# springmeyer/cov-tiles

Hardware: AMD Instinct MI355X
Metric: GB/s raw COVT bytes decoded + Mvertices/s, z2–z14 tile batch, 1/2/4/8 GPU (higher is better)
Workload: dtype int32

## Files before the change

cov-tiles_amd/__init__.py:

```python
from __future__ import annotations

import ctypes as C
import os
import subprocess
from dataclasses import dataclass
from typing import List, Optional

import numpy as np

_HERE = os.path.dirname(os.path.abspath(__file__))
_LIB = os.path.join(_HERE, os.environ.get("COVT_LIB_VARIANT", "libcovt.so"))

OK = 0
ERR_UNSUPPORTED_ENCODING = -1
ERR_TRUNCATED = -2
ERR_COUNT_MISMATCH = -3
ERR_BAD_HEADER = -4
ERR_DEVICE = -5
ERR_INVALID_ARG = -6
INPUT_PADDING = 4096
FORMAT_GENC, FORMAT_GEND = 0, 1
FAMILY_RLE, FAMILY_VARINT, FAMILY_FASTPFOR, FAMILY_LANE, FAMILY_SPLIT, FAMILY_SPLIT_FPF, FAMILY_SPLIT_RLE = range(7)
NUM_FAMILIES = 7
DESC_LANE, DESC_SPLIT, DESC_SPLIT_PAD, DESC_SPLIT_FPF = 0x1, 0x2, 0x4, 0x8
DESC_SPLIT_RLE = 0x10
SPLIT_SLOTS = 8
ID_FORMAT, ID_JAVA = 0, 1
LAUNCH_AUTO, LAUNCH_FUSED, LAUNCH_FORKED = 0, 1, 2
LAUNCH_FPF_STREAM, LAUNCH_FPF_CLASSIC = 0x4, 0x8

(OP_NONE, OP_BYTE_RLE_U8, OP_RLE_U64, OP_RLE_I32, OP_RLE_S64, OP_VARINT_I32, OP_VARINT_ZZ_I32,
 OP_VARINT_ZZ_DELTA_I32, OP_VARINT_ZZ_DELTA_XY, OP_VARINT_DELTA_MORTON, OP_FPF_ZZ_DELTA_I32, OP_FPF_ZZ_DELTA_XY,
 OP_FPF_DELTA_MORTON, OP_VARINT_U64, OP_VARINT_I32_AS_I64, OP_VARINT_ZZ_DELTA_I64, OP_BYTE_RLE_RAW,
 OP_VARINT_ZZ_I32_AS_I64, OP_VARINT_ZZ_S64, OP_VARINT_ZZ_DELTA_S64) = range(20)

PLAN_PROPERTIES = 0x1
RELEASE_PINNED = 0x2
PROP_BOOLEAN, PROP_INT64, PROP_FLOAT, PROP_STRING = 0, 1, 2, 3
PROP_DICT_OWNER, PROP_DENSE_BOOL, PROP_UNSUPPORTED, PROP_DATA_SHORT, PROP_UNSUPPORTED_LATE = 0x1, 0x2, 0x4, 0x8, 0x10

GEOMETRY_TYPES, GEOMETRY_OFFSETS, PART_OFFSETS, RING_OFFSETS, VERTEX_OFFSETS, VERTEX_BUFFER = range(4, 10)


class CovtError(Exception):
    status = 0


class IllegalArgumentException(CovtError, ValueError):
    pass


class ArrayIndexOutOfBoundsException(CovtError, IndexError):
# ... 1007 lines not shown
```

cov-tiles_amd/csrc/covt_decode.hip:

```cpp
#include <hip/hip_runtime.h>
#include <stdint.h>

#include "covt.h"
#include "covt_internal.h"
#include "covt_wave.h"
#include "covt_walk.h"

namespace covt {

constexpr int kWin = 1024;
constexpr int kFpfBlock = 256;
constexpr int kFpfPage = 65536;
constexpr int kFpfBcCap = 3 * kFpfPage / kFpfBlock + kFpfPage;

#ifndef COVT_LONG_STREAM
#define COVT_LONG_STREAM 16384
#endif
#ifndef COVT_LONG_PRIO
#define COVT_LONG_PRIO 2
#endif
#ifndef COVT_RLE_SHORT_SPAN
#define COVT_RLE_SHORT_SPAN 448
#endif
#ifndef COVT_CHUNK_PRIO
// ... 2039 lines not shown
    if ((cx | cy) == 0u) return;
    __builtin_amdgcn_s_waitcnt(0x0f70);
    int32_t* o = (int32_t*)out;
    typedef __attribute__((address_space(1))) i32x4 g_i4;
    const int32_t nq = (v1 - v0) >> 2;
    const int32_t last = v0 + 4 * (nq > 0 ? nq - 1 : 0);
    constexpr int kDeep = 8;
    for (int32_t q0 = 0; q0 < nq; q0 += 64 * kDeep) {
        i32x4 v[kDeep];
#pragma unroll
        for (int k = 0; k < kDeep; ++k) v[k] = *(const g_i4*)(o + min(v0 + 4 * (q0 + 64 * k + lane_id()), last));
#pragma unroll
        for (int k = 0; k < kDeep; ++k) {
            const int32_t q = q0 + 64 * k + lane_id();
            if (q < nq)
                st_out16(o + v0 + 4 * q, make_int4((int32_t)((uint32_t)v[k].x + cx), (int32_t)((uint32_t)v[k].y + cy),
                                                   (int32_t)((uint32_t)v[k].z + cx), (int32_t)((uint32_t)v[k].w + cy)));
        }
    }
    const int32_t i = v0 + 4 * nq + lane_id();
    if (i < v1) o[i] = (int32_t)((uint32_t)o[i] + (((i - v0) & 1) ? cy : cx));
}

constexpr int kSplitSlots = COVT_SPLIT_SLOTS;
struct Agg {
    int32_t cnt;
    uint32_t sx, sy;
};
__device__ __forceinline__ Agg agg_cat(const Agg& a, const Agg& b, bool xy) {
    if (a.cnt < 0) return a;
    if (b.cnt < 0) return Agg{b.cnt, b.sx, (uint32_t)a.cnt + b.sy};
    const bool sw = xy && (a.cnt & 1);
    return Agg{a.cnt + b.cnt, a.sx + (sw ? b.sy : b.sx), a.sy + (sw ? b.sx : b.sy)};
}
typedef __attribute__((address_space(1))) uint64_t g_u64;
__device__ __forceinline__ void rec_publish(covt_stream_result* rec, const Agg& a, uint32_t tag) {
    if (lane_id() == 0) {
        g_u64* g = (g_u64*)rec;
        const uint64_t t = (uint64_t)tag << 32;
        __hip_atomic_store(g, t | (uint32_t)a.cnt, __ATOMIC_RELAXED, __HIP_MEMORY_SCOPE_AGENT);
        __hip_atomic_store(g + 1, t | a.sx, __ATOMIC_RELAXED, __HIP_MEMORY_SCOPE_AGENT);
        __hip_atomic_store(g + 2, t | a.sy, __ATOMIC_RELAXED, __HIP_MEMORY_SCOPE_AGENT);
    }
}
__device__ __forceinline__ bool rec_try(covt_stream_result* rec, uint32_t tag, Agg& a) {
    g_u64* g = (g_u64*)rec;
// ... 298 lines not shown
                                                                           covt_stream_result* __restrict__ res) {
    constexpr int kStride = K == kSplitFpf ? kFamSmemFpf : K == kSplitRle ? kFamSmemRle : kFamSmemVarint;
    __shared__ __attribute__((aligned(16))) uint8_t smem[kWavesPerBlock * kStride];
    const int wv = uni((int)(threadIdx.x >> 6));
#ifdef COVT_TIMING
    const uint64_t t_start = __builtin_amdgcn_s_memrealtime();
#endif
    const int64_t t = decode_split_chunk<K>((WaveSmem*)(smem + wv * kStride), in, descs, n_chunks, out, res);
#ifdef COVT_TIMING
    if (t >= 0 && covt_phase_buf && lane_id() == 0) {
        const uint64_t t_end = __builtin_amdgcn_s_memrealtime();
        uint32_t* row = covt_phase_buf + (descs + kSplitSlots * t - covt_phase_desc0) * kPhases;
        row[0] = (uint32_t)(t_end - t_start);
        row[1] = (uint32_t)t_start;
    }
#else
    (void)t;
#endif
}

template <int FAM, bool FS = false>
__device__ __forceinline__ void decode_family_wave(uint8_t* smem, const uint8_t* __restrict__ in,
                                                   const covt_stream_desc* __restrict__ descs, int64_t sid,
                                                   uint8_t* __restrict__ out, covt_stream_result* __restrict__ res) {
    const covt_stream_desc d = descs[sid];
    if ((d.flags & (COVT_DESC_LANE | COVT_DESC_SPLIT | COVT_DESC_SPLIT_PAD)) || op_family(d.op) != FAM) return;
    if (d.byte_length > kLongStream || d.num_values > kLongStream) __builtin_amdgcn_s_setprio(COVT_LONG_PRIO);
#ifdef COVT_TIMING
    const uint64_t t_start = __builtin_amdgcn_s_memrealtime();
#endif
    Ctx c;
    c.sm = (WaveSmem*)smem;
    c.sb = in + d.in_off;
    c.out = out + d.out_off;
    c.avail = d.avail;
    c.n = d.num_values;
    c.nb = d.num_bits;
    c.op = d.op;
    c.byte_length = d.byte_length;
    c.err = 0;
    c.consumed = 0;
#ifdef COVT_TIMING
    c.ph_last = __builtin_amdgcn_s_memtime();
    for (int k = 0; k < kPhases; ++k) c.ph[k] = 0;
#endif
    if (c.n < 0 || c.avail < 0 || c.byte_length < 0) {
        c.err = COVT_ERR_INVALID_ARG;
    } else if (FAM == COVT_FAMILY_RLE) {
        if (c.op == COVT_OP_BYTE_RLE_U8 || c.op == COVT_OP_BYTE_RLE_RAW) { if (c.n > 0) run_rle_byte(c); }
// ... 40 lines not shown
        r.status = c.err;
        r.consumed = c.consumed;
#ifdef COVT_TIMING
        const uint64_t t_end = __builtin_amdgcn_s_memrealtime();
        r.status = c.err ? -1 : (int32_t)(t_end - t_start);
        r.consumed = (int32_t)(uint32_t)t_start;
        if (covt_phase_buf)
            for (int k = 0; k < kPhases; ++k) covt_phase_buf[(descs + sid - covt_phase_desc0) * kPhases + k] = c.ph[k];
#endif
        res[sid] = r;
    }
}

#ifndef COVT_FPF_WAVES
#define COVT_FPF_WAVES 7
#endif
#ifndef COVT_FPF_STREAM_WAVES
#define COVT_FPF_STREAM_WAVES 8
#endif
template <int FAM, bool FS = false>
__global__ __launch_bounds__(64 * kWavesPerBlock) __attribute__((amdgpu_waves_per_eu(FAM == COVT_FAMILY_FASTPFOR ? (FS ? COVT_FPF_STREAM_WAVES : COVT_FPF_WAVES) : 7))) void decode_family_kernel(const uint8_t* __restrict__ in,
                                                            const covt_stream_desc* __restrict__ descs,
                                                            int64_t n_streams, uint8_t* __restrict__ out,
                                                            covt_stream_result* __restrict__ res) {
    constexpr int kStride = FAM == COVT_FAMILY_RLE ? kFamSmemRle
                            : FAM == COVT_FAMILY_VARINT ? kFamSmemVarint : kFamSmemFpf;
    __shared__ __attribute__((aligned(16))) uint8_t smem[kWavesPerBlock * kStride];
    const int wv = uni((int)(threadIdx.x >> 6));
    const int64_t sid = (int64_t)blockIdx.x * kWavesPerBlock + wv;
    if (sid >= n_streams) return;
    decode_family_wave<FAM, FS>(smem + wv * kStride, in, descs, sid, out, res);
}

#ifndef COVT_LANE_SLOT
#define COVT_LANE_SLOT 17
#endif
constexpr int kLaneSlot = COVT_LANE_SLOT;
static_assert(kLaneSlot % 4 == 1, "16-byte granules plus one dword");
struct LaneBytes {
    const uint8_t* sb;
    uint32_t* slot;
    int32_t avail;
    int32_t w0;
    int32_t cq;
    uint32_t cw;
    __device__ __forceinline__ void load(int32_t p) {
        const uintptr_t a = (uintptr_t)(sb + p), a4 = a & ~(uintptr_t)3;
        w0 = p - (int32_t)(a & 3u);
        const int32_t need = avail - w0;
        uint32_t st[kLaneSlot];
#pragma unroll
        for (int k = 0; k < kLaneSlot / 4; ++k) {
            u32x4 v = {0u, 0u, 0u, 0u};
            if (16 * k < need) v = *(const __attribute__((address_space(1))) u32x4*)(a4 + 16 * k);
// ... 335 lines not shown
        sg.n[f] = counts[f];
        off += counts[f];
    }
    uint64_t wg = 0;
    for (int k = 0; k < COVT_NUM_FAMILIES; ++k) {
        const int f = covt::kFusedOrder[k];
        const int64_t n = f == COVT_FAMILY_SPLIT || f == COVT_FAMILY_SPLIT_FPF || f == COVT_FAMILY_SPLIT_RLE
                              ? counts[f] / covt::kSplitSlots : counts[f];
        const int64_t per = f == COVT_FAMILY_LANE ? 64 * kWavesPerBlock : kWavesPerBlock;
        wg += (uint64_t)((n + per - 1) / per);
        if (wg > 0x7fffffffull) return COVT_ERR_INVALID_ARG;
        sg.wg_end[k] = (uint32_t)wg;
    }
    if (wg == 0) return COVT_OK;
    hipLaunchKernelGGL(covt::decode_fused_kernel, dim3((unsigned)wg), dim3(64 * kWavesPerBlock), 0, stream,
                       d_in, d_out, sg);
    return hipGetLastError() == hipSuccess ? COVT_OK : COVT_ERR_DEVICE;
}

extern "C" int covt_launch_family_split_mode(int fam, const uint8_t* d_in, const covt_stream_desc* d_desc,
                                             int64_t n_streams, uint8_t* d_out, covt_stream_result* d_res,
                                             const covt_stream_desc* d_split, int64_t n_split,
                                             covt_stream_result* d_split_res, hipStream_t stream, int fpf_mode) {
    if (fpf_mode != 0 && fpf_mode != COVT_LAUNCH_FPF_STREAM && fpf_mode != COVT_LAUNCH_FPF_CLASSIC)
        return COVT_ERR_INVALID_ARG;
    if (n_split < 0 || n_split % covt::kSplitSlots) return COVT_ERR_INVALID_ARG;
    if (n_split && fam != COVT_FAMILY_VARINT && fam != COVT_FAMILY_FASTPFOR && fam != COVT_FAMILY_RLE)
        return COVT_ERR_INVALID_ARG;
    if (n_streams <= 0 && n_split == 0) return COVT_OK;
    if (n_streams < 0) n_streams = 0;
    if (fam == COVT_FAMILY_LANE) {
        const int64_t lblocks = (n_streams + 255) / 256;
        if (lblocks > 0x7fffffff) return COVT_ERR_INVALID_ARG;
        hipLaunchKernelGGL(covt::decode_lane_kernel, dim3((unsigned)lblocks), dim3(256), 0, stream, d_in, d_desc,
                           n_streams, d_out, d_res);
        return hipGetLastError() == hipSuccess ? COVT_OK : COVT_ERR_DEVICE;
    }
    const int64_t n_chunks = n_split / covt::kSplitSlots;
    const dim3 block(64 * kWavesPerBlock);
    if (n_chunks > 0) {
        const int64_t sblocks = (n_chunks + kWavesPerBlock - 1) / kWavesPerBlock;
        if (sblocks > 0x7fffffff) return COVT_ERR_INVALID_ARG;
        if (fam == COVT_FAMILY_FASTPFOR)
            hipLaunchKernelGGL(covt::decode_split_kernel<covt::kSplitFpf>, dim3((unsigned)sblocks), block, 0, stream,
                               d_in, d_split, n_chunks, d_out, d_split_res);
        else if (fam == COVT_FAMILY_RLE)
            hipLaunchKernelGGL(covt::decode_split_kernel<covt::kSplitRle>, dim3((unsigned)sblocks), block, 0, stream,
                               d_in, d_split, n_chunks, d_out, d_split_res);
        else
            hipLaunchKernelGGL(covt::decode_split_kernel<covt::kSplitVarint>, dim3((unsigned)sblocks), block, 0,
                               stream, d_in, d_split, n_chunks, d_out, d_split_res);
        if (hipGetLastError() != hipSuccess) return COVT_ERR_DEVICE;
    }
    if (n_streams <= 0) return COVT_OK;
    const int64_t blocks = (n_streams + kWavesPerBlock - 1) / kWavesPerBlock;
    if (blocks > 0x7fffffff) return COVT_ERR_INVALID_ARG;
    const dim3 grid((unsigned)blocks);
    switch (fam) {
    case COVT_FAMILY_RLE:
        hipLaunchKernelGGL(covt::decode_family_kernel<COVT_FAMILY_RLE>, grid, block, 0, stream, d_in, d_desc,
                           n_streams, d_out, d_res);
        break;
    case COVT_FAMILY_VARINT:
        hipLaunchKernelGGL(covt::decode_family_kernel<COVT_FAMILY_VARINT>, grid, block, 0, stream, d_in, d_desc,
                           n_streams, d_out, d_res);
        break;
    case COVT_FAMILY_FASTPFOR:
        if (fpf_mode == COVT_LAUNCH_FPF_STREAM || (fpf_mode == 0 && n_streams >= kFpfStreamMinStreams))
            hipLaunchKernelGGL((covt::decode_family_kernel<COVT_FAMILY_FASTPFOR, true>), grid, block, 0, stream, d_in,
                               d_desc, n_streams, d_out, d_res);
        else
            hipLaunchKernelGGL((covt::decode_family_kernel<COVT_FAMILY_FASTPFOR, false>), grid, block, 0, stream, d_in,
                               d_desc, n_streams, d_out, d_res);
        break;
    default: return COVT_ERR_INVALID_ARG;
    }
    return hipGetLastError() == hipSuccess ? COVT_OK : COVT_ERR_DEVICE;
}

extern "C" int covt_launch_family_split(int fam, const uint8_t* d_in, const covt_stream_desc* d_desc,
                                        int64_t n_streams, uint8_t* d_out, covt_stream_result* d_res,
                                        const covt_stream_desc* d_split, int64_t n_split, covt_stream_result* d_split_res,
                                        hipStream_t stream) {
    return covt_launch_family_split_mode(fam, d_in, d_desc, n_streams, d_out, d_res, d_split, n_split, d_split_res,
                                         stream, 0);
}

extern "C" int covt_launch_family(int fam, const uint8_t* d_in, const covt_stream_desc* d_desc, int64_t n_streams,
                                  uint8_t* d_out, covt_stream_result* d_res, hipStream_t stream) {
    return covt_launch_family_split(fam, d_in, d_desc, n_streams, d_out, d_res, nullptr, 0, nullptr, stream);
}

extern "C" int covt_op_family_of(int op) { return covt::op_family(op); }

#ifdef COVT_TIMING
extern "C" int covt_debug_set_phase_buffer(void* d_buf, const void* d_desc0) {
    if (hipMemcpyToSymbol(HIP_SYMBOL(covt::covt_phase_desc0), &d_desc0, sizeof(d_desc0)) != hipSuccess) return -5;
    return hipMemcpyToSymbol(HIP_SYMBOL(covt::covt_phase_buf), &d_buf, sizeof(d_buf)) == hipSuccess ? 0 : -5;
}
#endif
```

cov-tiles_amd/csrc/covt_host.cpp:

```cpp
#include <hip/hip_runtime.h>

#include <algorithm>
#include <atomic>
#include <cstdlib>
#include <cstring>
#include <sys/mman.h>
#include <memory>
#include <mutex>
#include <numeric>
#include <thread>
#include <unordered_map>
#include <vector>

#include "covt.h"
#include "covt_internal.h"
#include "covt_walk.h"
#include "covt_props_plan.h"

namespace {

bool name_is(const uint8_t* t, int64_t off, int64_t len, const char* s) {
    return (size_t)len == std::strlen(s) && std::memcmp(t + off, s, (size_t)len) == 0;
}

// ... 469 lines not shown
                return f;
            }
    }
    auto* f = new ForkCtx();
    f->device = dev;
    bool ok = true;
    for (int i = 0; i < kForkAux && ok; ++i)
        ok = hipStreamCreateWithFlags(&f->aux[i], hipStreamNonBlocking) == hipSuccess &&
             hipEventCreateWithFlags(&f->join[i], hipEventDisableTiming) == hipSuccess;
    if (ok) ok = hipEventCreateWithFlags(&f->fork, hipEventDisableTiming) == hipSuccess;
    if (!ok) {
        fork_destroy(f);
        return nullptr;
    }
    return f;
}
void fork_release(ForkCtx* f) {
    std::lock_guard<std::mutex> g(g_fork_mu);
    g_fork_free.push_back(f);
}

int launch_grouped(const uint8_t* d_in, const covt_stream_desc* d_desc, const int64_t counts[COVT_NUM_FAMILIES],
                   uint8_t* d_out, covt_stream_result* d_res, hipStream_t s, int mode = COVT_LAUNCH_AUTO) {
    const int fpf_mode = mode & (COVT_LAUNCH_FPF_STREAM | COVT_LAUNCH_FPF_CLASSIC);
    mode &= ~(COVT_LAUNCH_FPF_STREAM | COVT_LAUNCH_FPF_CLASSIC);
    if (fpf_mode == (COVT_LAUNCH_FPF_STREAM | COVT_LAUNCH_FPF_CLASSIC)) return COVT_ERR_INVALID_ARG;
    if (mode != COVT_LAUNCH_AUTO && mode != COVT_LAUNCH_FUSED && mode != COVT_LAUNCH_FORKED) return COVT_ERR_INVALID_ARG;
    int dev = 0;
    if (hipGetDevice(&dev) != hipSuccess) return COVT_ERR_DEVICE;
    if (s) {
        int sdev = -1;
        if (hipStreamGetDevice(s, &sdev) != hipSuccess || sdev != dev) return COVT_ERR_DEVICE;
    }
    ForkCtx* fp = fork_acquire(dev);
    if (!fp) return COVT_ERR_DEVICE;
    struct Back { ForkCtx* f; ~Back() { fork_release(f); } } back{fp};
    ForkCtx& f = *fp;
    int64_t off[COVT_NUM_FAMILIES];
    off[0] = 0;
    for (int k = 1; k < COVT_NUM_FAMILIES; ++k) off[k] = off[k - 1] + counts[k - 1];
    constexpr int kSplitV = COVT_FAMILY_SPLIT, kSplitF = COVT_FAMILY_SPLIT_FPF, kSplitR = COVT_FAMILY_SPLIT_RLE;
    const int64_t n_split = counts[kSplitV] + counts[kSplitF] + counts[kSplitR];
    const bool splits = n_split > 0;
    auto n_of = [&](int fam) { return fam < 0 ? 0 : counts[fam]; };
    struct Q {
        int fam[3];
    };
    Q qs[4];
    int nq = 0;
    auto add = [&](int a, int b2, int c3) {
        Q q{{-1, -1, -1}};
        int k = 0;
        for (int f : {a, b2, c3})
            if (n_of(f) > 0) q.fam[k++] = f;
        if (k) qs[nq++] = q;
    };
    if (splits && hipMemsetAsync(d_res + off[kSplitV], 0, (size_t)n_split * sizeof(covt_stream_result), s) != hipSuccess)
        return COVT_ERR_DEVICE;
    {
        const int64_t waves = n_split / COVT_SPLIT_SLOTS + counts[COVT_FAMILY_FASTPFOR] + counts[COVT_FAMILY_RLE] +
                              counts[COVT_FAMILY_VARINT] +
                              (counts[COVT_FAMILY_LANE] + kFusedLaneStreams - 1) / kFusedLaneStreams;
        if (mode == COVT_LAUNCH_FUSED || (mode == COVT_LAUNCH_AUTO && waves <= kFusedMaxWaves))
            return covt_launch_fused(d_in, d_desc, counts, d_out, d_res, s);
    }
    if (splits) {
        add(kSplitV, COVT_FAMILY_VARINT, kSplitR);
        add(COVT_FAMILY_FASTPFOR, -1, -1);
        add(COVT_FAMILY_RLE, COVT_FAMILY_LANE, -1);
        add(kSplitF, -1, -1);
    } else {
        for (int f : {COVT_FAMILY_FASTPFOR, COVT_FAMILY_VARINT, COVT_FAMILY_RLE, COVT_FAMILY_LANE}) add(f, -1, -1);
    }
    if (nq > 1 && hipEventRecord(f.fork, s) != hipSuccess) return COVT_ERR_DEVICE;
    int st = COVT_OK;
    int nforked = 0;
    for (int i = 0; i < nq && !st; ++i) {
        hipStream_t q = s;
        if (i > 0) {
            q = f.aux[i - 1];
            if (hipStreamWaitEvent(q, f.fork, 0) != hipSuccess) return COVT_ERR_DEVICE;
            nforked = i;
        }
        for (int k = 0; k < 3 && !st; ++k) {
            const int fam = qs[i].fam[k];
            if (fam < 0) continue;
            if (fam != kSplitV && fam != kSplitF && fam != kSplitR) {
                st = covt_launch_family_split_mode(fam, d_in, d_desc + off[fam], counts[fam], d_out, d_res + off[fam],
                                                   nullptr, 0, nullptr, q, fpf_mode);
                continue;
            }
            const int kind = fam == kSplitV ? COVT_FAMILY_VARINT : fam == kSplitR ? COVT_FAMILY_RLE : COVT_FAMILY_FASTPFOR;
            st = covt_launch_family_split(kind, d_in, nullptr, 0, d_out, nullptr, d_desc + off[fam], counts[fam],
                                          d_res + off[fam], q);
        }
    }
    for (int i = 0; i < nforked; ++i) {
        if (hipEventRecord(f.join[i], f.aux[i]) != hipSuccess) return COVT_ERR_DEVICE;
        if (hipStreamWaitEvent(s, f.join[i], 0) != hipSuccess) return COVT_ERR_DEVICE;
    }
    return st;
}

}

namespace {

struct Prefault {
    std::vector<std::thread> th;
// ... 1254 lines not shown
```

cov-tiles_amd/csrc/covt_internal.h:

```cpp
#ifndef COVT_INTERNAL_H
#define COVT_INTERNAL_H

#include <hip/hip_runtime.h>
#include <stdint.h>

#include "covt.h"

extern "C" {
int covt_launch_family(int fam, const uint8_t* d_in, const covt_stream_desc* d_desc, int64_t n_streams,
                       uint8_t* d_out, covt_stream_result* d_res, hipStream_t stream);
int covt_launch_family_split(int fam, const uint8_t* d_in, const covt_stream_desc* d_desc, int64_t n_streams,
                             uint8_t* d_out, covt_stream_result* d_res, const covt_stream_desc* d_split,
                             int64_t n_split, covt_stream_result* d_split_res, hipStream_t stream);
int covt_launch_family_split_mode(int fam, const uint8_t* d_in, const covt_stream_desc* d_desc, int64_t n_streams,
                                  uint8_t* d_out, covt_stream_result* d_res, const covt_stream_desc* d_split,
                                  int64_t n_split, covt_stream_result* d_split_res, hipStream_t stream, int fpf_mode);
int covt_op_family_of(int op);
int covt_launch_fused(const uint8_t* d_in, const covt_stream_desc* d_desc, const int64_t counts[COVT_NUM_FAMILIES],
                      uint8_t* d_out, covt_stream_result* d_res, hipStream_t stream);
}
constexpr int64_t kFpfStreamMinStreams = 65536;
constexpr int64_t kFusedMaxWaves = 4096;
#ifndef COVT_WAVES_PER_BLOCK
#define COVT_WAVES_PER_BLOCK 2
#endif
constexpr int kWavesPerBlock = COVT_WAVES_PER_BLOCK;
constexpr int64_t kFusedLaneStreams = 64 * kWavesPerBlock;

constexpr int64_t kOutAlign = 128;
__host__ __device__ inline int64_t align_out(int64_t x) { return (x + kOutAlign - 1) & ~(kOutAlign - 1); }

constexpr int kLaunchFamShift = 13;
__host__ __device__ inline uint32_t lane_op_index(int32_t op) {
    return op == COVT_OP_BYTE_RLE_U8 ? 0u : op == COVT_OP_RLE_U64 ? 1u : op == COVT_OP_RLE_I32 ? 2u
         : op == COVT_OP_RLE_S64 ? 3u : 4u;
}
__host__ __device__ inline uint32_t launch_key(uint32_t fam, bool lane, int32_t op, int64_t cost) {
    const uint64_t c = cost > 0 ? (uint64_t)cost : 0;
    uint32_t sub;
    if (lane) {
        sub = (lane_op_index(op) << 10) | (1023u - (uint32_t)(c < 1023 ? c : 1023));
    } else {
        uint32_t h = 0;
        if (c) {
// ... 57 lines not shown
```

include/covt.h:

```cpp
#ifndef COVT_H
#define COVT_H

#include <stddef.h>
#include <stdint.h>

#ifdef __cplusplus
extern "C" {
#endif

#define COVT_OK 0
#define COVT_ERR_UNSUPPORTED_ENCODING (-1)
#define COVT_ERR_TRUNCATED (-2)
#define COVT_ERR_COUNT_MISMATCH (-3)
#define COVT_ERR_BAD_HEADER (-4)
#define COVT_ERR_DEVICE (-5)
#define COVT_ERR_INVALID_ARG (-6)

#define COVT_INPUT_PADDING 4096

#define COVT_FORMAT_GENC 0
#define COVT_FORMAT_GEND 1

#define COVT_ID_FORMAT 0
#define COVT_ID_JAVA 1
// ... 121 lines not shown
                     int32_t n_tiles, int32_t format, int32_t id_mode, covt_plan** out);
void covt_plan_destroy(covt_plan* plan);
int64_t covt_plan_num_streams(const covt_plan* plan);
int64_t covt_plan_output_bytes(const covt_plan* plan);
int covt_plan_totals(const covt_plan* plan, int64_t* in_bytes, int64_t* out_bytes, int64_t* vertices);
int covt_plan_streams(const covt_plan* plan, covt_stream_info* out);
int64_t covt_plan_num_descs(const covt_plan* plan);
int covt_plan_descs(const covt_plan* plan, covt_stream_desc* out);
int covt_plan_desc_streams(const covt_plan* plan, int64_t* out);
int covt_plan_family_counts(const covt_plan* plan, int64_t counts[COVT_NUM_FAMILIES]);
int covt_plan_tile_status(const covt_plan* plan, int32_t* out);

int covt_decode_streams_device(const uint8_t* d_in, const covt_stream_desc* d_desc, int64_t n_streams,
                               uint8_t* d_out, covt_stream_result* d_res, void* hip_stream);

int covt_decode_streams_device_grouped(const uint8_t* d_in, const covt_stream_desc* d_desc,
                                       const int64_t family_counts[COVT_NUM_FAMILIES], uint8_t* d_out,
                                       covt_stream_result* d_res, void* hip_stream);
#define COVT_LAUNCH_AUTO 0
#define COVT_LAUNCH_FUSED 1
#define COVT_LAUNCH_FORKED 2
#define COVT_LAUNCH_FPF_STREAM 0x4
#define COVT_LAUNCH_FPF_CLASSIC 0x8
int covt_decode_streams_device_grouped_mode(const uint8_t* d_in, const covt_stream_desc* d_desc,
                                            const int64_t family_counts[COVT_NUM_FAMILIES], uint8_t* d_out,
                                            covt_stream_result* d_res, void* hip_stream, int32_t launch_mode);

int covt_plan_decode_host(const covt_plan* plan, const uint8_t* bytes, uint64_t n_bytes, uint8_t* host_out,
                          covt_stream_result* host_res);

int covt_plan_decode_host_multi(const covt_plan* plan, const uint8_t* bytes, uint64_t n_bytes, int32_t n_gpus,
                                uint8_t* host_out, covt_stream_result* host_res);

int covt_plan_decode_host_shards(const covt_plan* plan, const uint8_t* bytes, uint64_t n_bytes, int32_t n_shards,
                                 const int32_t* shard_devices, uint8_t* host_out, covt_stream_result* host_res);

int covt_plan_release_device(const covt_plan* plan);

#define COVT_GEOM_CLOSED_IN_STREAM 0x1u
#define COVT_GEOM_TOO_LARGE 0x80000000u

typedef struct covt_geom_desc {
    int64_t in_off[6];
    int32_t in_len[6];
    int32_t in_res[6];
    int64_t out_off[6];
// ... 136 lines not shown
```

Before: 610.6.

## Add cooperative multi-wave FastPFOR decode for large streams with auto launch selection

Adds a FastPFOR kernel where a whole workgroup of several waves decodes one large stream. Wave 0 parses page and block headers into shared LDS batches, and all waves then unpack 256-value blocks and apply exceptions in parallel. The host launcher picks this path automatically when the FastPFOR family is small and there are no split FPF streams, and schedules it first on the forked queues. The aim is to cut the tail latency of single large FastPFOR streams decoded by one wave. The cost is workgroup barriers, serialized header parsing on one wave, and higher LDS use per workgroup.

```diff
diff --git a/cov-tiles_amd/__init__.py b/cov-tiles_amd/__init__.py
--- a/cov-tiles_amd/__init__.py
+++ b/cov-tiles_amd/__init__.py
@@ -28,6 +28,7 @@
 ID_FORMAT, ID_JAVA = 0, 1
 LAUNCH_AUTO, LAUNCH_FUSED, LAUNCH_FORKED = 0, 1, 2
 LAUNCH_FPF_STREAM, LAUNCH_FPF_CLASSIC = 0x4, 0x8
+LAUNCH_FPF_COOP, LAUNCH_FPF_NOCOOP = 0x10, 0x20
 
 (OP_NONE, OP_BYTE_RLE_U8, OP_RLE_U64, OP_RLE_I32, OP_RLE_S64, OP_VARINT_I32, OP_VARINT_ZZ_I32,
  OP_VARINT_ZZ_DELTA_I32, OP_VARINT_ZZ_DELTA_XY, OP_VARINT_DELTA_MORTON, OP_FPF_ZZ_DELTA_I32, OP_FPF_ZZ_DELTA_XY,
diff --git a/cov-tiles_amd/csrc/covt_decode.hip b/cov-tiles_amd/csrc/covt_decode.hip
--- a/cov-tiles_amd/csrc/covt_decode.hip
+++ b/cov-tiles_amd/csrc/covt_decode.hip
@@ -2085,6 +2085,409 @@
     if (i < v1) o[i] = (int32_t)((uint32_t)o[i] + (((i - v0) & 1) ? cy : cx));
 }
 
+#ifndef COVT_FPF_COOP_WAVES
+#define COVT_FPF_COOP_WAVES 8
+#endif
+constexpr int kCoopWaves = COVT_FPF_COOP_WAVES;
+static_assert(kCoopWaves >= 2 && kCoopWaves <= 16, "cooperative FastPFOR workgroup: 2..16 waves");
+struct __attribute__((aligned(16))) CoopSmem {
+    WaveSmem w0;
+    uint32_t stage[kCoopWaves][328];
+    uint32_t patch[kCoopWaves][256];
+    int32_t rb[64], rce[64], ridx[64], rpk[64], rbcoff[64];
+    uint32_t rxcur[64];
+    int32_t xs[64];
+    uint32_t tot[2][kCoopWaves][2];
+    int32_t page[4];
+    int32_t bat[4];
+};
+static_assert(2 * sizeof(CoopSmem) <= 160 * 1024 && sizeof(CoopSmem) <= 64 * 1024,
+              "two cooperative FastPFOR workgroups per CU (160 KiB of LDS)");
+
+template <int OP>
+__device__ __forceinline__ void run_fastpfor_coop(Ctx& c, CoopSmem& cs, const int w) {
+    WaveSmem& sm = cs.w0;
+    const int l = lane_id();
+    const Words W{c.sb, c.byte_length / 4};
+    const int32_t nw32 = W.nw;
+    const uint32_t sbmis = (uint32_t)((uintptr_t)c.sb & 15);
+    const uint32_t bsel = be_sel(sbmis & 3u);
+    const g_u8* sb4 = (const g_u8*)(((uintptr_t)c.sb) & ~(uintptr_t)3);
+    Carry cr{0u, 0u};
+    uint32_t sc = 0;
+    int32_t L = 0, p = 1, done = 0, mw0 = 0;
+    int xs_v = 0, xz_v = -1, xc_v = 0;
+    uint32_t head1 = 0;
+    if (w == 0) {
+        if (c.byte_length > c.avail) c.err = COVT_ERR_TRUNCATED;
+        if (!c.err && nw32 > 0) {
+            const uint32_t head0 = W.uniform(0);
+            head1 = W.uniform(1);
+            L = (int32_t)head0;
+            if (L < 0) c.err = COVT_ERR_BAD_HEADER;
+            L -= L % kFpfBlock;
+            if (!c.err && L > c.n) c.err = COVT_ERR_COUNT_MISMATCH;
+        }
+    }
+    const uintptr_t s_end = (uintptr_t)c.sb + 4u * (uint32_t)nw32;
+    struct WordsRaw {
+        uint4 r;
+        int32_t base;
+        uint32_t sh;
+    };
+    auto words_issue = [&](int32_t wd) -> WordsRaw {
+        const uintptr_t addr = (uintptr_t)c.sb + 4u * (uint32_t)wd;
+        const uintptr_t a16 = addr & ~(uintptr_t)15;
+        const uint32_t o = (uint32_t)(addr & 15u);
+        const uint32_t lmax = s_end > a16 ? (uint32_t)((s_end - 1 - a16) >> 4) : 0u;
+        WordsRaw q;
+        q.r = ld128_off((const g_u8*)a16, 16u * min((uint32_t)l, lmax));
+        q.base = uni(wd - (int32_t)(o >> 2));
+        q.sh = o & 3u;
+        return q;
+    };
+    auto words_store = [&](uint32_t* dst, const WordsRaw& q) -> int32_t {
+        const uint32_t nx = lane_next(q.r.x);
+        const uint32_t sel = be_sel(q.sh);
+        const int32_t wl = q.base + 4 * l;
+        uint4 wv;
+        wv.x = wl < nw32 ? be_word(q.r.y, q.r.x, sel) : 0u;
+        wv.y = wl + 1 < nw32 ? be_word(q.r.z, q.r.y, sel) : 0u;
+        wv.z = wl + 2 < nw32 ? be_word(q.r.w, q.r.z, sel) : 0u;
+        wv.w = wl + 3 < nw32 ? be_word(nx, q.r.w, sel) : 0u;
+        wave_sync();
+        ((uint4*)dst)[l] = wv;
+        wave_sync();
+        return q.base;
+    };
+    auto load_words = [&](uint32_t* dst, int32_t wd) -> int32_t { return words_store(dst, words_issue(wd)); };
+    int32_t ie = 0, nblocks = 0, bclen = 0, bc = 0, cbase = 0, cur = 0, pk = 0;
+    bool xin = false;
+    auto chunk_load = [&](int32_t at) { cbase = (int32_t)(4 * (load_words(sm.u.f.cbuf, bc + (at >> 2)) - bc)); };
+    for (;;) {
+        if (w == 0) {
+            int32_t go = 0;
+            do {
+                if (c.err || nw32 <= 0 || done >= L) break;
+                done = uni(done);
+                const int32_t thissize = uni((L - done) < kFpfPage ? (L - done) : kFpfPage);
+                const int32_t p0 = uni(p);
+                if (p0 >= nw32) { c.err = COVT_ERR_TRUNCATED; break; }
+                const int64_t ie0 = (int64_t)p0 + (int32_t)(p0 == 1 ? head1 : W.uniform(p0));
+                if (ie0 < 0 || ie0 >= nw32) { c.err = COVT_ERR_TRUNCATED; break; }
+                ie = (int32_t)ie0;
+                mw0 = load_words(sm.u.f.cbuf, ie);
+                auto mword = [&](int32_t wd) -> uint32_t { return uniu(sm.u.f.cbuf[wd - mw0]); };
+                const int32_t bytesize = (int32_t)mword(ie++);
+                if (bytesize < 0 || bytesize > kFpfBcCap) { c.err = COVT_ERR_BAD_HEADER; break; }
+                xc_v = 0;
+                const int32_t bcw = (bytesize + 3) / 4;
+                bc = ie;
+                if (bc + bcw >= nw32) { c.err = COVT_ERR_TRUNCATED; break; }
+                ie += bcw;
+                int64_t ie64 = ie;
+                {
+                    int32_t dbase = INT32_MIN / 2;
+                    auto dword = [&](int32_t wd) -> uint32_t {
+                        if (wd >= mw0 && wd < mw0 + 255) return mword(wd);
+                        if (wd < dbase || wd >= dbase + 255) dbase = load_words(sm.u.f.ring, wd);
+                        return uniu(sm.u.f.ring[wd - dbase]);
+                    };
+                    uint32_t bm = dword((int32_t)ie64++) & ~1u;
+                    xs_v = 0;
+                    xz_v = -1;
+                    while (bm) {
+                        const int32_t k = __builtin_ctz(bm) + 1;
+                        bm &= bm - 1;
+                        if (ie64 >= nw32) { c.err = COVT_ERR_TRUNCATED; break; }
+                        const int32_t size = (int32_t)dword((int32_t)ie64++);
+                        if (size < 0) { c.err = COVT_ERR_BAD_HEADER; break; }
+                        const int64_t groups = ((int64_t)size + 31) / 32;
+                        xs_v = l == k ? (int)(uint32_t)ie64 : xs_v;
+                        xz_v = l == k ? size : xz_v;
+                        ie64 += groups * k;
+                        ie64 -= ((groups * 32 - size) * k) / 32;
+                    }
+                    if (c.err) break;
+                }
+                xin = ie64 - mw0 <= 255;
+                ie = (int32_t)(ie64 < nw32 ? ie64 : (int64_t)nw32);
+                nblocks = uni(thissize / kFpfBlock);
+                bclen = uni(bcw * 4);
+                cbase = (int32_t)(4 * (mw0 - bc));
+                cur = 0;
+                pk = p0 + 1;
+                cs.xs[l] = xs_v;
+                go = 1;
+            } while (false);
+            if (l == 0) {
+                cs.page[0] = go;
+                cs.page[1] = done;
+                cs.page[2] = bc;
+            }
+        }
+        __syncthreads();
+        if (uni(cs.page[0]) == 0) break;
+        const int32_t pdone = uni(cs.page[1]);
+        const g_u8* cbyte = (const g_u8*)(c.sb + 4u * (uint32_t)uni(cs.page[2]));
+        int32_t jbat = 0;
+        for (;;) {
+            if (w == 0) {
+                jbat = uni(jbat);
+                int32_t nbat = uni(min(64, nblocks - jbat));
+                uint32_t hw_v = 0u;
+                int32_t cur_v = bclen + 1;
+                cur = uni(cur);
+                cbase = uni(cbase);
+                if (!xin && cur <= bclen && (uint32_t)(cur - cbase) > (uint32_t)(1020 - 258)) chunk_load(cur);
+                for (int32_t g = 0; g < nbat; ++g) {
+                    cur = uni(cur);
+                    cbase = uni(cbase);
+                    if (cur > bclen) break;
+                    if (!xin && cur - cbase > 1020 - 8) {
+                        nbat = g;
+                        break;
+                    }
+                    const int32_t q = cur - cbase;
+                    const uint32_t hw =
+                        uniu(__builtin_amdgcn_alignbyte(sm.u.f.cbuf[(q >> 2) + 1], sm.u.f.cbuf[q >> 2], (uint32_t)q & 3u));
+                    const int32_t ce = (int32_t)((hw >> 8) & 0xffu);
+                    const int32_t nx = cur + (ce > 0 ? 3 + ce : 2);
+                    if (!xin && g > 0 && nx - cbase > 1020) {
+                        nbat = g;
+                        break;
+                    }
+                    hw_v = l == g ? hw : hw_v;
+                    cur_v = l == g ? cur : cur_v;
+                    cur = nx;
+                }
+                nbat = uni(nbat);
+                const bool in = l < nbat;
+                const int32_t b_v = (int32_t)(int8_t)(hw_v & 0xffu);
+                const int32_t ce_v = (int32_t)((hw_v >> 8) & 0xffu);
+                const bool hasx = ce_v > 0;
+                const int32_t idx_v = hasx ? (int32_t)(int8_t)((hw_v >> 16) & 0xffu) - b_v : 1;
+                const bool arr_k = hasx && idx_v >= 2 && idx_v <= 32;
+                const bool arr = in && arr_k;
+                int32_t xcur_v = 0;
+                for (uint64_t todo = __ballot(arr); todo;) {
+                    const int32_t kk = __builtin_amdgcn_readlane(idx_v, (int32_t)__builtin_ctzll(todo));
+                    const bool mine = arr && idx_v == kk;
+                    const uint32_t v = mine ? (uint32_t)ce_v : 0u;
+                    const uint32_t s = incl_scan(v);
+                    const int32_t base = __builtin_amdgcn_readlane(xc_v, kk);
+                    xcur_v = mine ? base + (int32_t)(s - v) : xcur_v;
+                    xc_v += l == kk ? (int32_t)lane_bcast(s, 63) : 0;
+                    todo &= ~__ballot(mine);
+                }
+                const uint32_t w8 = in ? 8u * (uint32_t)(b_v & 63) : 0u;
+                const uint32_t pinc = incl_scan(w8);
+                const int32_t pk_v = pk + (int32_t)(pinc - w8);
+                pk += (int32_t)lane_bcast(pinc, 63);
+                int32_t nok = nbat;
+                int32_t ferr = nbat == 0 ? COVT_ERR_BAD_HEADER : 0;
+                {
+                    const int32_t xsz = lane_get(xz_v, arr_k ? idx_v : 0);
+                    bool bad = (uint32_t)b_v > 32u || cur_v + 2 > bclen;
+                    bad |= hasx && (cur_v + 3 + ce_v > bclen || (idx_v != 1 && !arr_k));
+                    bad |= arr_k && (xsz < 0 || xcur_v + ce_v > xsz);
+                    const bool trunc = pk_v + 8 * b_v > nw32;
+                    const uint64_t fail = __ballot(in && (bad || trunc));
+                    if (fail) {
+                        nok = (int32_t)__builtin_ctzll(fail);
+                        ferr = __builtin_amdgcn_readlane(bad ? COVT_ERR_BAD_HEADER : COVT_ERR_TRUNCATED, nok);
+                    }
+                }
+                cs.rb[l] = b_v;
+                cs.rce[l] = ce_v;
+                cs.ridx[l] = idx_v;
+                cs.rpk[l] = pk_v;
+                cs.rbcoff[l] = cur_v + (hasx ? 3 : 2);
+                cs.rxcur[l] = (uint32_t)xcur_v;
+                if (ferr) c.err = ferr;
+                if (l == 0) {
+                    cs.bat[0] = jbat;
+                    cs.bat[1] = nok;
+                    cs.bat[2] = ferr;
+                    cs.bat[3] = (ferr != 0 || jbat + nbat >= nblocks) ? 1 : 0;
+                }
+                jbat += nbat;
+            }
+            __syncthreads();
+            const int32_t j0 = uni(cs.bat[0]), nok = uni(cs.bat[1]);
+            const bool last = uni(cs.bat[3]) != 0;
+            struct Pre {
+                uint4 raw;
+                uint32_t pos, x0, x1, x2;
+            };
+            auto issue = [&](int32_t g, Pre& pr) {
+                const int32_t b = uni(cs.rb[g]), ce = uni(cs.rce[g]), k = uni(cs.ridx[g]);
+                const int32_t pkc = uni(cs.rpk[g]), bcoff = uni(cs.rbcoff[g]);
+                const uint32_t xcur = uniu(cs.rxcur[g]);
+                const uintptr_t a16 = ((uintptr_t)c.sb + 4u * (uint32_t)pkc) & ~(uintptr_t)15;
+                pr.raw = ld128_off((const g_u8*)a16, 16u * min((uint32_t)l, 2u * (uint32_t)b + 1u));
+                pr.pos = pr.x0 = pr.x1 = pr.x2 = 0u;
+                if (ce > 0) {
+                    pr.pos = cbyte[(uint32_t)(bcoff + min(l, ce - 1)) ^ 3u];
+                    if (k != 1) {
+                        const uint32_t xs = (uint32_t)uni(cs.xs[k]);
+                        const int32_t wx = (int32_t)(xs + (__umul24(xcur + (uint32_t)l, (uint32_t)k) >> 5));
+                        const uint32_t wi = l < ce && wx < nw32 ? (uint32_t)wx : 0u;
+                        const u32x3 xv = *(const g_v3*)(sb4 + 4u * wi);
+                        pr.x0 = xv.x;
+                        pr.x1 = xv.y;
+                        pr.x2 = xv.z;
+                    }
+                }
+            };
+            Pre pr;
+            pr.raw = make_uint4(0, 0, 0, 0);
+            pr.pos = pr.x0 = pr.x1 = pr.x2 = 0u;
+            if (w < nok) issue(w, pr);
+            for (int32_t g0 = 0; g0 < nok; g0 += kCoopWaves, ++sc) {
+                const int32_t g = g0 + w;
+                const bool act = g < nok;
+                const int64_t vbase = (int64_t)pdone + (int64_t)(j0 + g) * kFpfBlock;
+                uint32_t v[4] = {0u, 0u, 0u, 0u};
+                uint32_t tx = 0u, ty = 0u;
+                if (act) {
+                    const int32_t b = uni(cs.rb[g]), ce = uni(cs.rce[g]), k = uni(cs.ridx[g]);
+                    const int32_t pkc = uni(cs.rpk[g]), bcoff = uni(cs.rbcoff[g]);
+                    const uint32_t xcur = uniu(cs.rxcur[g]);
+                    uint32_t* stage = cs.stage[w];
+                    uint32_t* patch = cs.patch[w];
+                    const uintptr_t a16 = ((uintptr_t)c.sb + 4u * (uint32_t)pkc) & ~(uintptr_t)15;
+                    const uint4 raw = pr.raw;
+                    const bool el = l < ce;
+                    const uint32_t pos = pr.pos, x0 = pr.x0, x1 = pr.x1, x2 = pr.x2;
+                    uint32_t xbit = 0u;
+                    int32_t wx = 0;
+                    if (ce > 0 && k != 1) {
+                        const uint32_t bb = __umul24(xcur + (uint32_t)l, (uint32_t)k);
+                        xbit = bb & 31u;
+                        wx = (int32_t)((uint32_t)uni(cs.xs[k]) + (bb >> 5));
+                    }
+                    const int32_t qoff = (int32_t)(((sbmis + 4u * (uint32_t)pkc) & 15u) >> 2);
+                    {
+                        uint4 raw2 = make_uint4(0, 0, 0, 0);
+                        if (b == 32) raw2 = sld128(a16 + 1024);
+                        const uint32_t nxt = lane_next(raw.x, raw2.x);
+                        uint4 wv;
+                        wv.x = be_word(raw.y, raw.x, bsel);
+                        wv.y = be_word(raw.z, raw.y, bsel);
+                        wv.z = be_word(raw.w, raw.z, bsel);
+                        wv.w = be_word(nxt, raw.w, bsel);
+                        ((uint4*)stage)[l] = wv;
+                        if (b == 32 && l == 0) {
+                            uint4 w2;
+                            w2.x = be_word(raw2.y, raw2.x, bsel);
+                            w2.y = be_word(raw2.z, raw2.y, bsel);
+                            w2.z = be_word(raw2.w, raw2.z, bsel);
+                            w2.w = be_word(0u, raw2.w, bsel);
+                            ((uint4*)stage)[64] = w2;
+                        }
+                    }
+                    if (ce > 0) ((uint4*)patch)[l] = make_uint4(0, 0, 0, 0);
+                    wave_sync();
+                    {
+                        const uint32_t mask = b == 32 ? 0xffffffffu : ((1u << b) - 1u);
+                        uint32_t bit = __umul24((uint32_t)(l & 7) * 4u, (uint32_t)b);
+                        const int32_t wb = (int32_t)__umul24((uint32_t)(l >> 3), (uint32_t)b) + qoff;
+#pragma unroll
+                        for (int q = 0; q < 4; ++q) {
+                            const int32_t wi = wb + (int32_t)(bit >> 5);
+                            const uint32_t lo = stage[wi], hi = stage[wi + 1];
+                            v[q] = __builtin_amdgcn_alignbit(hi, lo, bit & 31u) & mask;
+                            bit += (uint32_t)b;
+                        }
+                    }
+                    if (ce > 0) {
+                        uint32_t ex = 1u;
+                        if (k != 1) {
+                            const uint32_t lo = wx < nw32 ? be_word(x1, x0, bsel) : 0u;
+                            const uint32_t hi = wx + 1 < nw32 ? be_word(x2, x1, bsel) : 0u;
+                            const uint32_t m = k == 32 ? 0xffffffffu : ((1u << k) - 1u);
+                            ex = __builtin_amdgcn_alignbit(hi, lo, xbit) & m;
+                        }
+                        atomicOr(&patch[el ? pos : (uint32_t)(4 * l)], el ? ex << (b & 31) : 0u);
+                        if (ce > 64) {
+                            const uint32_t xs = k >= 2 ? (uint32_t)uni(cs.xs[k]) : 0u;
+                            for (int q = 1; q < 4; ++q) {
+                                const int32_t e = l + 64 * q;
+                                if (e < ce) {
+                                    const uint32_t ex2 = k == 1 ? 1u : xget(W, xs, k, xcur + (uint32_t)e);
+                                    const uint32_t ps = cbyte[(uint32_t)(bcoff + e) ^ 3u];
+                                    atomicOr(&patch[ps], ex2 << (b & 31));
+                                }
+                            }
+                        }
+                        wave_sync();
+                        const uint4 pt = ((const uint4*)patch)[l];
+                        v[0] |= pt.x;
+                        v[1] |= pt.y;
+                        v[2] |= pt.z;
+                        v[3] |= pt.w;
+                    }
+                    if (g + kCoopWaves < nok) issue(g + kCoopWaves, pr);
+                    uint32_t ax = 0u, ay = 0u;
+                    sum_values<OP, 4>(v, vbase, kFpfBlock, ax, ay);
+                    tx = lane_bcast(incl_scan(ax), 63);
+                    if (OP == COVT_OP_FPF_ZZ_DELTA_XY) ty = lane_bcast(incl_scan(ay), 63);
+                    if (l == 0) {
+                        cs.tot[sc & 1u][w][0] = tx;
+                        cs.tot[sc & 1u][w][1] = ty;
+                    }
+                }
+                __syncthreads();
+                const int32_t cnt = min(kCoopWaves, nok - g0);
+                uint32_t px = cr.x, py = cr.y;
+#pragma unroll
+                for (int i = 0; i < kCoopWaves; ++i) {
+                    const uint32_t ux = uniu(cs.tot[sc & 1u][i][0]), uy = uniu(cs.tot[sc & 1u][i][1]);
+                    px += i < w ? ux : 0u;
+                    py += i < w ? uy : 0u;
+                    cr.x += i < cnt ? ux : 0u;
+                    cr.y += i < cnt ? uy : 0u;
+                }
+                if (act) {
+                    Carry cc{px, py};
+                    sink_values<OP, 4>(v, vbase, 0, kFpfBlock, c.nb, c.out, cc);
+                }
+            }
+            __syncthreads();
+            if (last) break;
+        }
+        if (w == 0) {
+            done += min(L - done, kFpfPage);
+            p = ie;
+        }
+    }
+    if (w != 0) return;
+    int32_t decoded = L;
+    if (!c.err && nw32 > 0 && p < nw32) {
+        int32_t vpos = (int32_t)(4 * p);
+        const int32_t base = L;
+        Win wn;
+        wn.valid = false;
+        const bool tail_in = L > 0 && ((vpos & ~15) >> 2) >= mw0 && nw32 - mw0 <= 255;
+        const int32_t got = varint_take<MODE_WORDREV, VAL_VB>(
+            sm, c.sb, wn, vpos, 4 * nw32, c.n - L, true, c.err,
+            [&](const uint32_t (&lo)[1], const uint32_t (&hi)[1], int32_t vb, int32_t, int32_t count) {
+                sink_values<OP, 1>(lo, (int64_t)base + vb, 0, count, c.nb, c.out, cr);
+            },
+            0, nullptr, 0, tail_in ? sm.u.f.cbuf : nullptr, (int32_t)mw0);
+        decoded = L + got;
+    }
+    if (!c.err) {
+        for (int32_t b = decoded; b < c.n; b += 64) {
+            uint32_t vv[1] = {0};
+            sink_values<OP, 1>(vv, b, 0, c.n - b < 64 ? c.n - b : 64, c.nb, c.out, cr);
+        }
+        if (OP == COVT_OP_FPF_ZZ_DELTA_XY && (c.n & 1)) c.err = COVT_ERR_COUNT_MISMATCH;
+    }
+    c.consumed = c.byte_length;
+}
+
 constexpr int kSplitSlots = COVT_SPLIT_SLOTS;
 struct Agg {
     int32_t cnt;
@@ -2429,9 +2832,11 @@
 template <int FAM, bool FS = false>
 __device__ __forceinline__ void decode_family_wave(uint8_t* smem, const uint8_t* __restrict__ in,
                                                    const covt_stream_desc* __restrict__ descs, int64_t sid,
-                                                   uint8_t* __restrict__ out, covt_stream_result* __restrict__ res) {
+                                                   uint8_t* __restrict__ out, covt_stream_result* __restrict__ res,
+                                                   int64_t coop_n = 0, int32_t coop_min = 0) {
     const covt_stream_desc d = descs[sid];
     if ((d.flags & (COVT_DESC_LANE | COVT_DESC_SPLIT | COVT_DESC_SPLIT_PAD)) || op_family(d.op) != FAM) return;
+    if (FAM == COVT_FAMILY_FASTPFOR && sid < coop_n && d.num_values >= coop_min) return;
     if (d.byte_length > kLongStream || d.num_values > kLongStream) __builtin_amdgcn_s_setprio(COVT_LONG_PRIO);
 #ifdef COVT_TIMING
     const uint64_t t_start = __builtin_amdgcn_s_memrealtime();
@@ -2518,14 +2923,73 @@
 __global__ __launch_bounds__(64 * kWavesPerBlock) __attribute__((amdgpu_waves_per_eu(FAM == COVT_FAMILY_FASTPFOR ? (FS ? COVT_FPF_STREAM_WAVES : COVT_FPF_WAVES) : 7))) void decode_family_kernel(const uint8_t* __restrict__ in,
                                                             const covt_stream_desc* __restrict__ descs,
                                                             int64_t n_streams, uint8_t* __restrict__ out,
-                                                            covt_stream_result* __restrict__ res) {
+                                                            covt_stream_result* __restrict__ res,
+                                                            int64_t coop_n, int32_t coop_min) {
     constexpr int kStride = FAM == COVT_FAMILY_RLE ? kFamSmemRle
                             : FAM == COVT_FAMILY_VARINT ? kFamSmemVarint : kFamSmemFpf;
     __shared__ __attribute__((aligned(16))) uint8_t smem[kWavesPerBlock * kStride];
     const int wv = uni((int)(threadIdx.x >> 6));
     const int64_t sid = (int64_t)blockIdx.x * kWavesPerBlock + wv;
     if (sid >= n_streams) return;
-    decode_family_wave<FAM, FS>(smem + wv * kStride, in, descs, sid, out, res);
+    decode_family_wave<FAM, FS>(smem + wv * kStride, in, descs, sid, out, res, coop_n, coop_min);
+}
+
+template <bool SPLIT>
+__global__ __launch_bounds__(64 * kCoopWaves) __attribute__((amdgpu_waves_per_eu(8))) void decode_fpf_coop_kernel(
+    const uint8_t* __restrict__ in, const covt_stream_desc* __restrict__ descs, uint8_t* __restrict__ out,
+    covt_stream_result* __restrict__ res, int32_t min_values) {
+    __shared__ CoopSmem cs;
+    const int64_t at = SPLIT ? (int64_t)blockIdx.x * kSplitSlots : (int64_t)blockIdx.x;
+    const covt_stream_desc d = descs[at];
+    if (SPLIT) {
+        if ((d.flags & (COVT_DESC_SPLIT | COVT_DESC_SPLIT_PAD)) != COVT_DESC_SPLIT || d.avail != 0) return;
+    } else {
+        if ((d.flags & (COVT_DESC_LANE | COVT_DESC_SPLIT | COVT_DESC_SPLIT_PAD)) ||
+            op_family(d.op) != COVT_FAMILY_FASTPFOR || d.num_values < min_values)
+            return;
+    }
+    const int w = uni((int)(threadIdx.x >> 6));
+    __builtin_amdgcn_s_setprio(COVT_LONG_PRIO);
+#ifdef COVT_TIMING
+    const uint64_t t_start = __builtin_amdgcn_s_memrealtime();
+#endif
+    Ctx c;
+    c.sm = &cs.w0;
+    c.sb = in + d.in_off;
+    c.out = out + d.out_off;
+    c.avail = SPLIT ? d.byte_length : d.avail;
+    c.n = d.num_values;
+    c.nb = d.num_bits;
+    c.op = d.op;
+    c.byte_length = d.byte_length;
+    c.err = 0;
+    c.consumed = 0;
+#ifdef COVT_TIMING
+    c.ph_last = __builtin_amdgcn_s_memtime();
+    for (int k = 0; k < kPhases; ++k) c.ph[k] = 0;
+#endif
+    if (c.n < 0 || c.avail < 0 || c.byte_length < 0) {
+        c.err = COVT_ERR_INVALID_ARG;
+    } else {
+        switch (c.op) {
+        case COVT_OP_FPF_ZZ_DELTA_I32: run_fastpfor_coop<COVT_OP_FPF_ZZ_DELTA_I32>(c, cs, w); break;
+        case COVT_OP_FPF_ZZ_DELTA_XY: run_fastpfor_coop<COVT_OP_FPF_ZZ_DELTA_XY>(c, cs, w); break;
+        default: run_fastpfor_coop<COVT_OP_FPF_DELTA_MORTON>(c, cs, w); break;
+        }
+    }
+    if (w == 0 && lane_id() == 0) {
+        covt_stream_result r;
+        r.status = c.err;
+        r.consumed = c.consumed;
+#ifdef COVT_TIMING
+        if (!SPLIT) {
+            const uint64_t t_end = __builtin_amdgcn_s_memrealtime();
+            r.status = c.err ? -1 : (int32_t)(t_end - t_start);
+            r.consumed = (int32_t)(uint32_t)t_start;
+        }
+#endif
+        res[at] = r;
+    }
 }
 
 #ifndef COVT_LANE_SLOT
@@ -2907,6 +3371,9 @@
                                              int64_t n_streams, uint8_t* d_out, covt_stream_result* d_res,
                                              const covt_stream_desc* d_split, int64_t n_split,
                                              covt_stream_result* d_split_res, hipStream_t stream, int fpf_mode) {
+    const int64_t coop_n = covt_fpf_coop_count(fpf_mode, fam == COVT_FAMILY_FASTPFOR ? n_streams : 0);
+    const int32_t coop_min = covt_fpf_coop_min(fpf_mode);
+    fpf_mode &= ~(COVT_LAUNCH_FPF_COOP | kFpfCoopAuto);
     if (fpf_mode != 0 && fpf_mode != COVT_LAUNCH_FPF_STREAM && fpf_mode != COVT_LAUNCH_FPF_CLASSIC)
         return COVT_ERR_INVALID_ARG;
     if (n_split < 0 || n_split % covt::kSplitSlots) return COVT_ERR_INVALID_ARG;
@@ -2944,19 +3411,19 @@
     switch (fam) {
     case COVT_FAMILY_RLE:
         hipLaunchKernelGGL(covt::decode_family_kernel<COVT_FAMILY_RLE>, grid, block, 0, stream, d_in, d_desc,
-                           n_streams, d_out, d_res);
+                           n_streams, d_out, d_res, (int64_t)0, 0);
         break;
     case COVT_FAMILY_VARINT:
         hipLaunchKernelGGL(covt::decode_family_kernel<COVT_FAMILY_VARINT>, grid, block, 0, stream, d_in, d_desc,
-                           n_streams, d_out, d_res);
+                           n_streams, d_out, d_res, (int64_t)0, 0);
         break;
     case COVT_FAMILY_FASTPFOR:
         if (fpf_mode == COVT_LAUNCH_FPF_STREAM || (fpf_mode == 0 && n_streams >= kFpfStreamMinStreams))
             hipLaunchKernelGGL((covt::decode_family_kernel<COVT_FAMILY_FASTPFOR, true>), grid, block, 0, stream, d_in,
-                               d_desc, n_streams, d_out, d_res);
+                               d_desc, n_streams, d_out, d_res, coop_n, coop_min);
         else
             hipLaunchKernelGGL((covt::decode_family_kernel<COVT_FAMILY_FASTPFOR, false>), grid, block, 0, stream, d_in,
-                               d_desc, n_streams, d_out, d_res);
+                               d_desc, n_streams, d_out, d_res, coop_n, coop_min);
         break;
     default: return COVT_ERR_INVALID_ARG;
     }
@@ -2976,6 +3443,20 @@
     return covt_launch_family_split(fam, d_in, d_desc, n_streams, d_out, d_res, nullptr, 0, nullptr, stream);
 }
 
+extern "C" int covt_launch_fpf_coop(int split, const uint8_t* d_in, const covt_stream_desc* d_desc, int64_t n,
+                                    uint8_t* d_out, covt_stream_result* d_res, int32_t min_values, hipStream_t stream) {
+    if (n <= 0) return COVT_OK;
+    if (n > 0x7fffffff) return COVT_ERR_INVALID_ARG;
+    const dim3 block(64 * covt::kCoopWaves);
+    if (split)
+        hipLaunchKernelGGL(covt::decode_fpf_coop_kernel<true>, dim3((unsigned)n), block, 0, stream, d_in, d_desc, d_out,
+                           d_res, min_values);
+    else
+        hipLaunchKernelGGL(covt::decode_fpf_coop_kernel<false>, dim3((unsigned)n), block, 0, stream, d_in, d_desc, d_out,
+                           d_res, min_values);
+    return hipGetLastError() == hipSuccess ? COVT_OK : COVT_ERR_DEVICE;
+}
+
 extern "C" int covt_op_family_of(int op) { return covt::op_family(op); }
 
 #ifdef COVT_TIMING
diff --git a/cov-tiles_amd/csrc/covt_host.cpp b/cov-tiles_amd/csrc/covt_host.cpp
--- a/cov-tiles_amd/csrc/covt_host.cpp
+++ b/cov-tiles_amd/csrc/covt_host.cpp
@@ -515,10 +515,20 @@
 
 int launch_grouped(const uint8_t* d_in, const covt_stream_desc* d_desc, const int64_t counts[COVT_NUM_FAMILIES],
                    uint8_t* d_out, covt_stream_result* d_res, hipStream_t s, int mode = COVT_LAUNCH_AUTO) {
-    const int fpf_mode = mode & (COVT_LAUNCH_FPF_STREAM | COVT_LAUNCH_FPF_CLASSIC);
-    mode &= ~(COVT_LAUNCH_FPF_STREAM | COVT_LAUNCH_FPF_CLASSIC);
-    if (fpf_mode == (COVT_LAUNCH_FPF_STREAM | COVT_LAUNCH_FPF_CLASSIC)) return COVT_ERR_INVALID_ARG;
+    constexpr int kFpfFlags = COVT_LAUNCH_FPF_STREAM | COVT_LAUNCH_FPF_CLASSIC | COVT_LAUNCH_FPF_COOP | COVT_LAUNCH_FPF_NOCOOP;
+    const int fpf_flags = mode & kFpfFlags;
+    mode &= ~kFpfFlags;
+    const int fpf_variant = fpf_flags & (COVT_LAUNCH_FPF_STREAM | COVT_LAUNCH_FPF_CLASSIC);
+    if (fpf_variant == (COVT_LAUNCH_FPF_STREAM | COVT_LAUNCH_FPF_CLASSIC)) return COVT_ERR_INVALID_ARG;
+    if ((fpf_flags & COVT_LAUNCH_FPF_COOP) && (fpf_flags & COVT_LAUNCH_FPF_NOCOOP)) return COVT_ERR_INVALID_ARG;
     if (mode != COVT_LAUNCH_AUTO && mode != COVT_LAUNCH_FUSED && mode != COVT_LAUNCH_FORKED) return COVT_ERR_INVALID_ARG;
+    if (fpf_flags && mode == COVT_LAUNCH_FUSED) return COVT_ERR_INVALID_ARG;
+    if (fpf_flags && mode == COVT_LAUNCH_AUTO) mode = COVT_LAUNCH_FORKED;
+    const bool coop_all = (fpf_flags & COVT_LAUNCH_FPF_COOP) != 0;
+    const bool coop = coop_all || (!(fpf_flags & COVT_LAUNCH_FPF_NOCOOP) && counts[COVT_FAMILY_FASTPFOR] > 0 &&
+                                   counts[COVT_FAMILY_FASTPFOR] < kFpfCoopMaxFamily &&
+                                   counts[COVT_FAMILY_SPLIT_FPF] == 0);
+    const int fpf_mode = fpf_variant | (fpf_flags & COVT_LAUNCH_FPF_COOP) | (coop ? kFpfCoopAuto : 0);
     int dev = 0;
     if (hipGetDevice(&dev) != hipSuccess) return COVT_ERR_DEVICE;
     if (s) {
@@ -535,7 +545,9 @@
     constexpr int kSplitV = COVT_FAMILY_SPLIT, kSplitF = COVT_FAMILY_SPLIT_FPF, kSplitR = COVT_FAMILY_SPLIT_RLE;
     const int64_t n_split = counts[kSplitV] + counts[kSplitF] + counts[kSplitR];
     const bool splits = n_split > 0;
-    auto n_of = [&](int fam) { return fam < 0 ? 0 : counts[fam]; };
+    constexpr int kCoopF = COVT_NUM_FAMILIES;
+    const int64_t n_coop = coop ? covt_fpf_coop_count(fpf_mode, counts[COVT_FAMILY_FASTPFOR]) : 0;
+    auto n_of = [&](int fam) { return fam < 0 ? 0 : fam == kCoopF ? n_coop : counts[fam]; };
     struct Q {
         int fam[3];
     };
@@ -557,13 +569,17 @@
         if (mode == COVT_LAUNCH_FUSED || (mode == COVT_LAUNCH_AUTO && waves <= kFusedMaxWaves))
             return covt_launch_fused(d_in, d_desc, counts, d_out, d_res, s);
     }
+    const bool coop_first = COVT_FPF_COOP_FIRST && (n_coop > 0 || (coop_all && counts[kSplitF] > 0));
     if (splits) {
+        if (coop_first) add(kSplitF, kCoopF, -1);
         add(kSplitV, COVT_FAMILY_VARINT, kSplitR);
         add(COVT_FAMILY_FASTPFOR, -1, -1);
         add(COVT_FAMILY_RLE, COVT_FAMILY_LANE, -1);
-        add(kSplitF, -1, -1);
+        if (!coop_first) add(kSplitF, kCoopF, -1);
     } else {
-        for (int f : {COVT_FAMILY_FASTPFOR, COVT_FAMILY_VARINT, COVT_FAMILY_RLE, COVT_FAMILY_LANE}) add(f, -1, -1);
+        if (coop_first) add(kCoopF, COVT_FAMILY_LANE, -1);
+        for (int f : {COVT_FAMILY_FASTPFOR, COVT_FAMILY_VARINT, COVT_FAMILY_RLE}) add(f, -1, -1);
+        if (!coop_first) add(kCoopF, COVT_FAMILY_LANE, -1);
     }
     if (nq > 1 && hipEventRecord(f.fork, s) != hipSuccess) return COVT_ERR_DEVICE;
     int st = COVT_OK;
@@ -578,6 +594,16 @@
         for (int k = 0; k < 3 && !st; ++k) {
             const int fam = qs[i].fam[k];
             if (fam < 0) continue;
+            if (fam == kCoopF) {
+                st = covt_launch_fpf_coop(0, d_in, d_desc + off[COVT_FAMILY_FASTPFOR], n_coop, d_out,
+                                          d_res + off[COVT_FAMILY_FASTPFOR], covt_fpf_coop_min(fpf_mode), q);
+                continue;
+            }
+            if (fam == kSplitF && coop_all) {
+                st = covt_launch_fpf_coop(1, d_in, d_desc + off[fam], counts[fam] / COVT_SPLIT_SLOTS, d_out,
+                                          d_res + off[fam], 0, q);
+                continue;
+            }
             if (fam != kSplitV && fam != kSplitF && fam != kSplitR) {
                 st = covt_launch_family_split_mode(fam, d_in, d_desc + off[fam], counts[fam], d_out, d_res + off[fam],
                                                    nullptr, 0, nullptr, q, fpf_mode);
diff --git a/cov-tiles_amd/csrc/covt_internal.h b/cov-tiles_amd/csrc/covt_internal.h
--- a/cov-tiles_amd/csrc/covt_internal.h
+++ b/cov-tiles_amd/csrc/covt_internal.h
@@ -16,10 +16,33 @@
                                   uint8_t* d_out, covt_stream_result* d_res, const covt_stream_desc* d_split,
                                   int64_t n_split, covt_stream_result* d_split_res, hipStream_t stream, int fpf_mode);
 int covt_op_family_of(int op);
+int covt_launch_fpf_coop(int split, const uint8_t* d_in, const covt_stream_desc* d_desc, int64_t n, uint8_t* d_out,
+                         covt_stream_result* d_res, int32_t min_values, hipStream_t stream);
 int covt_launch_fused(const uint8_t* d_in, const covt_stream_desc* d_desc, const int64_t counts[COVT_NUM_FAMILIES],
                       uint8_t* d_out, covt_stream_result* d_res, hipStream_t stream);
 }
 constexpr int64_t kFpfStreamMinStreams = 65536;
+#ifndef COVT_FPF_COOP_STREAMS
+#define COVT_FPF_COOP_STREAMS 1024
+#endif
+#ifndef COVT_FPF_COOP_MIN
+#define COVT_FPF_COOP_MIN 8192
+#endif
+#ifndef COVT_FPF_COOP_MAX_FAMILY
+#define COVT_FPF_COOP_MAX_FAMILY 32768
+#endif
+constexpr int64_t kFpfCoopMaxFamily = COVT_FPF_COOP_MAX_FAMILY;
+#ifndef COVT_FPF_COOP_FIRST
+#define COVT_FPF_COOP_FIRST 1
+#endif
+constexpr int64_t kFpfCoopStreams = COVT_FPF_COOP_STREAMS;
+constexpr int32_t kFpfCoopMin = COVT_FPF_COOP_MIN;
+constexpr int kFpfCoopAuto = 0x100;
+inline int64_t covt_fpf_coop_count(int fpf_mode, int64_t n_fpf) {
+    if (fpf_mode & COVT_LAUNCH_FPF_COOP) return n_fpf;
+    return (fpf_mode & kFpfCoopAuto) ? (n_fpf < kFpfCoopStreams ? n_fpf : kFpfCoopStreams) : 0;
+}
+inline int32_t covt_fpf_coop_min(int fpf_mode) { return (fpf_mode & COVT_LAUNCH_FPF_COOP) ? 256 : kFpfCoopMin; }
 constexpr int64_t kFusedMaxWaves = 4096;
 #ifndef COVT_WAVES_PER_BLOCK
 #define COVT_WAVES_PER_BLOCK 2
diff --git a/include/covt.h b/include/covt.h
--- a/include/covt.h
+++ b/include/covt.h
@@ -167,6 +167,8 @@
 #define COVT_LAUNCH_FORKED 2
 #define COVT_LAUNCH_FPF_STREAM 0x4
 #define COVT_LAUNCH_FPF_CLASSIC 0x8
+#define COVT_LAUNCH_FPF_COOP 0x10
+#define COVT_LAUNCH_FPF_NOCOOP 0x20
 int covt_decode_streams_device_grouped_mode(const uint8_t* d_in, const covt_stream_desc* d_desc,
                                             const int64_t family_counts[COVT_NUM_FAMILIES], uint8_t* d_out,
                                             covt_stream_result* d_res, void* hip_stream, int32_t launch_mode);
```

Result: no change. 608.6 (-0.3%).
